# NilanEkanayake/TiTok-Video

Measured on AMD Instinct MI355X. Metric: video clips/sec encode+decode (whole node), higher is better.
Workload: dtype bf16

## Files before the change

### include/titok_hip.h

```cpp
#ifndef TITOK_HIP_H
#define TITOK_HIP_H

#include <stdint.h>

#ifdef __cplusplus
extern "C" {
#endif

#define TTV_OK 0
#define TTV_ERR_INVALID 1
#define TTV_ERR_LAUNCH 2
#define TTV_ERR_UNSUPPORTED 3

#define TTV_BF16 0
#define TTV_F32 1

#define TTV_ENCODER 0
#define TTV_DECODER 1

#define TTV_MAX_FSQ 8
#define TTV_MAX_TOKEN 64
#define TTV_MAX_CLIPS_PER_LAUNCH 64

const char* ttv_error_string(void);
// ... 68 lines not shown

int64_t ttv_mlp_pack_bytes(int inner, int next_qkv_rows);
int ttv_mlp_pack(const void* w12_folded, const void* w3, const void* out_proj, const void* next_qkv_folded, int next_qkv_rows, int inner,
                 int width, int dtype, void* mlp_packed, void* stream);
int ttv_mlp_fused(const void* x, int ldx, const void* mlp_packed, int inner, void* y, int ldy, const float* post_gain, float alpha,
                  float eps, int M, int width, int dtype, void* stream);
typedef struct ttv_next_qkv {
  void* qkv; int32_t ld;
  const float* rope_cs;
  int32_t rows;
  int32_t rope_q_end, rope_k_begin, rope_k_end;
} ttv_next_qkv;
int ttv_layer_tail_fused(const void* ao, int ldao, const float* attn_post_gain, float attn_alpha, const void* x, int ldx,
                         const void* mlp_packed, int inner, void* y, int ldy, const float* ffd_post_gain, float ffd_alpha, float eps,
                         int M, int width, int dtype, const ttv_next_qkv* next, void* stream);

int ttv_fill_const_rows(void* x, int dtype, int ld, const int32_t* rows_map, int rows, int width, const float* mask_token,
                        const float* gain, float eps, void* stream);
int ttv_decoder_embed(const void* codes, int token_size, const void* w, const void* bias, const float* mask_token, const float* gain,
                      void* x, int dtype, int ld, const int32_t* rows_map, int rows, int width, float eps, void* stream);

#define TTV_ATTN_GATE 1
#define TTV_ATTN_PAIRED 2
#define TTV_ATTN_QSCALED 4
#define TTV_ATTN_ALLFULL 8
#define TTV_ATTN_PIPE 16
#define TTV_ATTN_SPLIT3 32
#define TTV_ATTN_SPLIT_OUT 64
#define TTV_ATTN_SPLIT_IN 128
int ttv_attention(const void* qkvg, int ld, void* out, int ldo, const int32_t* cu_seqlens, const int32_t* qblocks,
// ... 434 lines not shown
  TTV_DBG_GEMM_TILE128 = 256,
  TTV_DBG_GEMM_T256 = 512,
  TTV_DBG_MLP_TILES9 = 512,
  TTV_DBG_GEMM_NO_T256 = 1024,
  TTV_DBG_MX_UNFUSED_QUANT = 2048,
  TTV_DBG_SPLIT3_NO_IMAGES = 4096,
  TTV_DBG_SPLIT3_NO_DMA = 8192,
  TTV_DBG_K256_GENERAL = 16384,
  TTV_DBG_QKV256_OFF = 32768,
  TTV_DBG_QKV256_WS = 131072,
  TTV_DBG_ENC_ALL_ROWS = 524288,
  TTV_DBG_ATTN_NO_SWP = 1048576,
  TTV_DBG_DEC_ALL_BLOCKS = 2097152,
  TTV_DBG_DEC_L0_NO_CONST = 4194304,
  TTV_DBG_ENC_LAST_QKV_ALL = 8388608,
  TTV_DBG_PATCH_EMBED_UNFUSED = 16777216
};
int ttv_debug_set(int flags);
int ttv_debug_stamps(void* device_buffer);
int ttv_prof_end(double* total_ms, int* count);

#ifdef __cplusplus
}
#endif
#endif
```

### titok_video_amd/_lib.py

```python
from __future__ import annotations

import ctypes as C
import os
import threading

import torch

from . import switches

TTV_BF16, TTV_F32 = 0, 1
TTV_ENCODER, TTV_DECODER = 0, 1
TTV_MAX_FSQ = 8
TTV_MAX_TOKEN = 64
TTV_MAX_CLIPS_PER_LAUNCH = 64
TTV_DISC_HEAD_GENERATOR, TTV_DISC_HEAD_DISCRIMINATOR = 0, 1
TTV_TAPE_STORED, TTV_TAPE_RECOMPUTE = 0, 1

DBG_NO_STORES = 1
DBG_K256_NO_PANEL_DMA = 2
DBG_MLP_NO_WEIGHT_DMA = 2
DBG_K256_NO_TILE_RELOAD = 4
DBG_MLP_NO_GEGLU = 4
DBG_K256_NO_EPILOGUE_MATH = 8
DBG_MLP_TILES8 = 8
# ... 5 lines not shown
DBG_GEMM_T256 = 512
DBG_MLP_TILES9 = 512
DBG_GEMM_NO_T256 = 1024
DBG_MX_UNFUSED_QUANT = 2048
DBG_SPLIT3_NO_IMAGES = 4096
DBG_SPLIT3_NO_DMA = 8192
DBG_K256_GENERAL = 16384
DBG_QKV256_OFF = 32768
DBG_QKV256_WS = 131072
DBG_ENC_ALL_ROWS = 524288
DBG_ATTN_NO_SWP = 1048576
DBG_DEC_ALL_BLOCKS = 2097152
DBG_DEC_L0_NO_CONST = 4194304
DBG_ENC_LAST_QKV_ALL = 8388608
DBG_PATCH_EMBED_UNFUSED = 16777216

_HERE = os.path.dirname(os.path.abspath(__file__))
LIB_PATH = switches.text("TTV_LIB_PATH") or os.path.join(_HERE, "libtitok_hip.so")

i32, i64, f32, vp = C.c_int32, C.c_int64, C.c_float, C.c_void_p


class FsqParams(C.Structure):
    _fields_ = [("n", i32), ("levels", i32 * TTV_MAX_FSQ), ("basis", i32 * TTV_MAX_FSQ),
                ("half_l", f32 * TTV_MAX_FSQ), ("offset", f32 * TTV_MAX_FSQ), ("shift", f32 * TTV_MAX_FSQ),
                ("half_width", f32 * TTV_MAX_FSQ)]


class TowerDims(C.Structure):
    _fields_ = [("kind", i32), ("dtype", i32), ("width", i32), ("layers", i32), ("q_heads", i32), ("kv_heads", i32),
# ... 150 lines not shown
    "ttv_linear_fp8_mx": (C.c_int, [vp, C.c_int, vp, vp, vp, C.c_int, vp, vp, vp, C.c_int, C.c_int, C.c_int, C.c_int, C.c_int, vp, C.c_int, C.c_int,
                                    vp, C.c_int, f32, vp]),
    "ttv_rmsnorm": (C.c_int, [vp, C.c_int, C.c_int, vp, vp, C.c_int, C.c_int, vp, vp, C.c_int, C.c_int, f32, vp]),
    "ttv_rope_apply": (C.c_int, [vp, C.c_int, C.c_int, C.c_int, C.c_int, vp, vp]),
    "ttv_linear": (C.c_int, [vp, C.c_int, vp, C.c_int, vp, vp, vp, C.c_int, C.c_int, C.c_int, C.c_int, C.c_int, vp]),
    "ttv_linear_qkv_rope": (C.c_int, [vp, C.c_int, vp, C.c_int, vp, C.c_int, C.c_int, C.c_int, C.c_int, vp, C.c_int, vp]),
    "ttv_linear_geglu": (C.c_int, [vp, C.c_int, vp, C.c_int, vp, C.c_int, C.c_int, C.c_int, C.c_int, C.c_int, vp]),
    "ttv_linear_residual": (C.c_int, [vp, C.c_int, vp, C.c_int, vp, C.c_int, f32, vp, C.c_int, C.c_int, C.c_int, C.c_int,
                                      C.c_int, C.c_int, vp]),
    "ttv_linear_residual_norm": (C.c_int, [vp, C.c_int, vp, C.c_int, vp, C.c_int, f32, vp, f32, vp, C.c_int, C.c_int, C.c_int,
                                           C.c_int, C.c_int, vp]),
    "ttv_mlp_pack_bytes": (C.c_int64, [C.c_int, C.c_int]),
    "ttv_mlp_pack": (C.c_int, [vp, vp, vp, vp, C.c_int, C.c_int, C.c_int, C.c_int, vp, vp]),
    "ttv_layer_tail_fused": (C.c_int, [vp, C.c_int, vp, f32, vp, C.c_int, vp, C.c_int, vp, C.c_int, vp, f32, f32, C.c_int, C.c_int,
                                       C.c_int, vp, vp]),
    "ttv_mlp_fused": (C.c_int, [vp, C.c_int, vp, C.c_int, vp, C.c_int, vp, f32, f32, C.c_int, C.c_int, C.c_int, vp]),
    "ttv_fill_const_rows": (C.c_int, [vp, C.c_int, C.c_int, vp, C.c_int, C.c_int, vp, vp, f32, vp]),
    "ttv_decoder_embed": (C.c_int, [vp, C.c_int, vp, vp, vp, vp, vp, C.c_int, C.c_int, vp, C.c_int, C.c_int, f32, vp]),
    "ttv_attention": (C.c_int, [vp, C.c_int, vp, C.c_int, vp, vp, C.c_int, C.c_int, C.c_int, C.c_int, C.c_int, C.c_int, vp]),
    "ttv_attention64": (C.c_int, [vp, C.c_int, vp, C.c_int, vp, vp, C.c_int, C.c_int, C.c_int, C.c_int, C.c_int, C.c_int, vp]),
    "ttv_rmsnorm_mx": (C.c_int, [vp, C.c_int, C.c_int, vp, C.c_int, C.c_int, vp, C.c_int, C.c_int, f32, vp, vp, vp, vp]),
    "ttv_attention_pv8_bytes": (C.c_int64, [C.c_int, C.c_int, C.c_int]),
    "ttv_quant_v_pv8": (C.c_int, [vp, C.c_int, vp, C.c_int, C.c_int, C.c_int, C.c_int, vp, vp]),
    "ttv_attention_pv8": (C.c_int, [vp, C.c_int, vp, C.c_int, vp, vp, C.c_int, C.c_int, C.c_int, C.c_int, C.c_int, vp, vp]),
    "ttv_attention_mxout": (C.c_int, [vp, C.c_int, vp, vp, C.c_int, vp, vp, C.c_int, C.c_int, C.c_int, vp]),
    "ttv_linear_fp8_mx_geglu_q": (C.c_int, [vp, C.c_int, vp, vp, vp, C.c_int, vp, vp, vp, vp, C.c_int, C.c_int, C.c_int, vp]),
    "ttv_row_rstd": (C.c_int, [vp, C.c_int, C.c_int, vp, C.c_int, C.c_int, f32, vp]),
    "ttv_linear_rowscale": (C.c_int, [vp, C.c_int, vp, C.c_int, vp, C.c_int, vp, C.c_int, C.c_int, vp, C.c_int, C.c_int, C.c_int, C.c_int, C.c_int, vp]),
    "ttv_patch_gather": (C.c_int, [C.POINTER(vp), vp, C.c_int, C.c_int, C.c_int, C.c_int, C.c_int, C.c_int, vp, C.c_int,
                                   C.c_int, C.c_int, vp]),
# ... 156 lines not shown
```

### titok_video_amd/csrc/ttv_api.hip

```cpp
#include <stdarg.h>
#include <stdio.h>
#include <stdlib.h>
#include <string.h>

#include "ttv_common.h"
#include "ttv_kernels.h"

static thread_local char g_err[512] = "";

void ttv_set_error(const char* fmt, ...) {
  va_list ap;
  va_start(ap, fmt);
  vsnprintf(g_err, sizeof(g_err), fmt, ap);
  va_end(ap);
}

int g_ttv_prof_class = 0;
bool ttv_sw_enc_latent_last() { static const bool v = ttv_env_flag("TTV_ENC_LATENT_LAST", true); return v; }
bool ttv_enc_latent_rows_only(const ttv_tower_dims* d, const ttv_batch* b) {
  return ttv_sw_enc_latent_last() && !(g_ttv_debug & TTV_DBG_ENC_ALL_ROWS) && d->kind == TTV_ENCODER && b->latent_rows && b->sum_tokens > 0 &&
         b->sum_tokens < b->total_rows;
}
bool ttv_sw_keel_f32sum() { static const bool v = ttv_env_flag("TTV_KEEL_F32SUM", false); return v; }
bool ttv_sw_fused_patch() { static const bool v = ttv_env_flag("TTV_FUSED_PATCH", true); return v; }
bool ttv_sw_attn_pipe() { static const bool v = ttv_env_flag("TTV_ATTN_PIPE", false); return v; }
static bool sw_dec_l0_const() { static const bool v = ttv_env_flag("TTV_DEC_L0_CONST", true); return v; }
static bool sw_enc_last_qkv_skip() { static const bool v = ttv_env_flag("TTV_ENC_LAST_QKV_SKIP", true); return v; }
float ttv_sw_attn_thr() { static const float v = ttv_env_float("TTV_ATTN_THR", 8.0f); return v; }
thread_local int g_ttv_debug = 0;
long long* g_ttv_stamps = nullptr;
static hipEvent_t* g_prof_start = nullptr;
static hipEvent_t* g_prof_stop = nullptr;
static int g_prof_cap = 0, g_prof_n = 0;

TtvProfScope::TtvProfScope(int cls, hipStream_t stream) : slot(-1), s(stream) {
  if (g_ttv_prof_class != 0 && cls == g_ttv_prof_class && g_prof_n < g_prof_cap) {
    slot = g_prof_n++;
    (void)hipEventRecord(g_prof_start[slot], s);
  }
}
TtvProfScope::~TtvProfScope() {
  if (slot >= 0) (void)hipEventRecord(g_prof_stop[slot], s);
}

struct TowerWs {
  char *x, *xn, *qkv, *ao, *h, *pa, *pb;
  char *xl, *aol;
  char *f8, *f8mx;
  float* y32;
  float* rstd;
  int64_t total;
};

static TowerWs carve(const ttv_tower_dims* d, const ttv_batch* b, char* base) {
  const int64_t e = dtype_bytes(d->dtype);
  const int64_t L = b->total_rows, P = b->sum_patches;
  const int64_t g = (int64_t)d->kv_heads * d->head_dim;
  const int64_t pd = patch_dim(d);
  int64_t off = 0;
  TowerWs w;
  auto take = [&](int64_t bytes) { char* p = base ? base + off : nullptr; off += align256(bytes); return p; };
  w.x = take(L * d->width * e);
  w.xn = take(L * d->width * e);
  w.qkv = take(L * (2 * d->width + 2 * g) * e);
  w.ao = take(L * d->width * e);
  w.y32 = (float*)take(L * d->width * 4);
  w.h = take(L * d->inner * e);
  w.pa = take(P * pd * e);
  w.pb = take(P * d->width * e);
  w.rstd = (float*)take(L * 4);
  w.xl = take((int64_t)b->sum_tokens * d->width * e);
  w.aol = take((int64_t)b->sum_tokens * d->width * e);
  w.f8 = w.f8mx = nullptr;
  if (d->dtype == TTV_BF16 && d->width != 256 && d->width % 128 == 0) {
    const int64_t wide = d->width > d->inner ? d->width : d->inner;
    w.f8 = take(L * wide);
    w.f8mx = take(L * (wide / 128 + 4) * 4);
  }
  w.total = off;
  return w;
}

static int check_dims(const ttv_tower_dims* d, const ttv_batch* b) {
  TTV_CHECK_ARG(d && b, "null dims/batch");
  TTV_CHECK_ARG(d->dtype == TTV_BF16 || d->dtype == TTV_F32, "bad dtype %d", d->dtype);
  TTV_CHECK_ARG(d->head_dim == 64 && d->width == d->q_heads * 64, "width must be q_heads*64");
  TTV_CHECK_ARG(d->width % 64 == 0 && d->width <= 1024, "width %d unsupported", d->width);
// ... 126 lines not shown
    return ttvk_gemm(EPI_RESID_NORM, o, c.s);
  }
  float* const next_rstd = want_rstd ? c.ws.rstd : nullptr;
  if (dt == TTV_BF16 && !ttv_sw_keel_f32sum()) {
    TTV_TRY(ttvk_gemm(EPI_RESID_T, o, c.s));
    TTV_TRY(ttvk_rmsnorm(cx, dt, dm, nullptr, cx, dt, dm, nullptr, post_gain, o.M, dm, d->eps, c.s, next_rstd));
  } else {
    o.y = c.ws.y32;
    TTV_TRY(ttvk_gemm(EPI_RESID_F32, o, c.s));
    TTV_TRY(ttvk_rmsnorm(c.ws.y32, TTV_F32, dm, nullptr, cx, dt, dm, nullptr, post_gain, o.M, dm, d->eps, c.s, next_rstd));
  }
  rstd_valid = want_rstd;
  return TTV_OK;
}

static bool qkv_tile_list_ok(const LayerCtx& c, const ttv_layer_weights& lw, int K, int P) {
  const ttv_tower_dims* d = c.d;
  const ttv_batch* b = c.b;
  if (d->dtype != TTV_BF16 || d->width != 256 || d->head_dim != 64 || c.split3) return false;
  if (K <= 0 || P <= 0 || K % 128 || P % 128 || (int64_t)b->n_clips * K != b->sum_tokens || (int64_t)b->n_clips * P != b->sum_patches) return false;
  if (!lw.to_qkv_pn || !lw.qkv_q_prescaled) return false;
  return ttvk_gemm_qkv_tiles_supported(d->width, d->kv_heads * d->head_dim, d->width);
}

static bool dec_l0_const_ok(const LayerCtx& c, const ttv_tower_weights* w, const ttv_dec_l0_const* l0) {
  const ttv_tower_dims* d = c.d;
  const ttv_batch* b = c.b;
  if (!l0 || !l0->rows || !sw_dec_l0_const() || (g_ttv_debug & TTV_DBG_DEC_L0_NO_CONST)) return false;
  if (d->kind != TTV_DECODER || !qkv_tile_list_ok(c, w->layers[0], l0->latent_rows, l0->patch_rows)) return false;
  if (c.pair || c.pipe || c.pv8 || !c.all_full || (b->items64 && b->n_items64 > 0)) return false;
  return ttvk_attention_takes_swp(TTV_ATTN_GATE | TTV_ATTN_QSCALED | TTV_ATTN_ALLFULL);
}

static bool enc_last_qkv_skip_ok(const LayerCtx& c, const ttv_layer_weights& lw) {
  const ttv_batch* b = c.b;
// ... 1 lines not shown
  return qkv_tile_list_ok(c, lw, b->tokens_per_clip, b->max_patches_per_clip);
}

static int run_layers(const ttv_tower_dims* d, const ttv_tower_weights* w, const ttv_batch* b, const TowerWs& ws, hipStream_t s,
                      const ttv_dec_l0_const* l0 = nullptr) {
  const int L = b->total_rows, dm = d->width, g = d->kv_heads * d->head_dim, dt = d->dtype;
  const int split3 = (dt == TTV_F32 && w->f32_split3) ? 1 : 0;
  const bool gen_ok = (dt == TTV_BF16 && dm != 256) || split3;
  static const bool s3img_env = ttv_env_flag("TTV_SPLIT3_IMAGES", true);
  const int s3img = (split3 && s3img_env && !(g_ttv_debug & TTV_DBG_SPLIT3_NO_IMAGES)) ? 1 : 0;
  const int nq = 2 * dm + 2 * g;
  const int64_t row_bytes = (int64_t)dm * dtype_bytes(dt);
  bool qkv_ready = false;
  bool rstd_valid = false;
  bool xq_valid = false;
  const bool lat_last = ttv_enc_latent_rows_only(d, b) && b->qblocks_latent && b->n_qblocks_latent > 0;
  static const bool pat_env = ttv_env_flag("TTV_DEC_PATCH_LAST", true);
  const bool pat_last = pat_env && !(g_ttv_debug & TTV_DBG_DEC_ALL_BLOCKS) && d->kind == TTV_DECODER && d->layers >= 2 && b->qblocks_patch &&
                        b->n_qblocks_patch > 0 && !split3 && !b->qblocks_paired;
  bool compacted = false;
  const bool pv8 = w->attn_pv8 != 0;
  TTV_CHECK_ARG(!pv8 || (dt == TTV_BF16 && !split3), "attn_pv8 is a bf16 inference option (not for fp32 or split-bf16 towers)");
  const LayerCtx ctx = {d, b, ws, s, split3, s3img, gen_ok, b->qblocks_paired ? TTV_ATTN_PAIRED : 0, b->qblocks_all_full ? TTV_ATTN_ALLFULL : 0,
                        ttv_sw_attn_pipe() ? TTV_ATTN_PIPE : 0, pv8};
  const bool l0_const = dec_l0_const_ok(ctx, w, l0);
  for (int i = 0; i < d->layers; ++i) {
    const ttv_layer_weights& lw = w->layers[i];
    const bool last = i == d->layers - 1;
    const bool l0c = l0_const && i == 0;
    if (dt == TTV_BF16 && dm != 256 && dm % 128 == 0 && d->inner % 128 == 0 && !ttv_sw_keel_f32sum() && lw.to_qkv_f8 && lw.to_qkv_mx && lw.w12_f8 &&
        lw.w12_mx && lw.out_proj_f8 && lw.out_proj_mx && lw.w3_f8 && lw.w3_mx &&
        !(lat_last && last)) {
      TTV_TRY(run_layer_mx(ctx, lw, i, rstd_valid, xq_valid));
      qkv_ready = false;
// ... 20 lines not shown
    else if (l0c) {
      TtvProfScope prof(TTV_KC_ATTENTION, s);
      const bool own = l0->qblocks && l0->n_qblocks > 0;
      TTV_TRY(ttvk_attention_swp(ws.qkv, nq, ws.ao, dm, b->cu_seqlens, own ? l0->qblocks : b->qblocks, own ? l0->n_qblocks : b->n_qblocks, d->q_heads,
                                 d->kv_heads, 1, s, l0->rows, l0->latent_rows, l0->state));
    } else if (pat_last && last && dt == TTV_BF16 && !ctx.pipe)
      TTV_TRY(tower_attention(ctx, q_scaled, b->qblocks_patch, b->n_qblocks_patch, ctx.all_full));
    else if (q_scaled && b->items64 && b->n_items64 > 0 && d->head_dim == 64 && !pv8)
      TTV_TRY(ttvk_attention64(ws.qkv, nq, ws.ao, dm, b->cu_seqlens, b->items64, b->n_items64, d->q_heads, d->kv_heads,
                               TTV_ATTN_GATE | TTV_ATTN_QSCALED, s));
    else
      TTV_TRY(tower_attention(ctx, q_scaled, b->qblocks, b->n_qblocks, ctx.pair | ctx.all_full | ctx.pipe));
    char* cx = ws.x;
    char* cao = ws.ao;
    int Lc = L;
    if (lat_now) {
      TTV_TRY(gather_rows(ws.x, ws.xl, b->latent_rows, b->sum_tokens, row_bytes, s));
      TTV_TRY(gather_rows(ws.ao, ws.aol, b->latent_rows, b->sum_tokens, row_bytes, s));
      cx = ws.xl; cao = ws.aol; Lc = b->sum_tokens;
      compacted = true;
    }
    static const bool use_fused_mlp = ttv_env_flag("TTV_FUSED_MLP", true);
    static const bool use_fused_qkv = ttv_env_flag("TTV_FUSED_QKV", false);
    const float alpha = keel_alpha(d, i);
    if (use_fused_mlp && ttvk_mlp_fused_supported(dt, dm, d->inner) && lw.mlp_pack) {
      MlpNextQkv nx = {};
      const bool back = use_fused_qkv && !last && lw.mlp_pack_qkv_rows == nq && nq % 64 == 0 && dm % 64 == 0 && g % 64 == 0;
      if (back) { nx.qkv = ws.qkv; nx.ld = nq; nx.rope_cs = b->rope_cs; nx.rows = nq; nx.rope_q_end = dm; nx.rope_k_begin = 2 * dm; nx.rope_k_end = 2 * dm + g; }
      TTV_TRY(ttvk_mlp_fused(cao, dm, i == 0 ? nullptr : lw.attn_post_ln, alpha, cx, dm, lw.mlp_pack, d->inner, cx, dm, i == 0 ? nullptr : lw.ffd_post_ln,
                             alpha, d->eps, Lc, back ? &nx : nullptr, s));
      qkv_ready = back;
      continue;
    }
    TTV_TRY(keel_tail(ctx, gemm_args(dt, cao, dm, lw.out_proj, dm, Lc, dm, dm, cx, dm), i, lw.attn_post_ln, gen_ok && lw.w12_pn && !f8_w12, rstd_valid));
    const PreNormW fw = {lw.ffd_norm, lw.w12, lw.w12_pn, lw.w12_f8, lw.w12_f8_scale, f8_w12};
    TTV_TRY(prenorm_proj(ctx, EPI_GEGLU, cx, Lc, fw, d->inner, ws.h, s3img, rstd_valid));
    rstd_valid = false;
    const ttv_layer_weights* nl = last ? nullptr : &w->layers[i + 1];
    const bool next_rstd = gen_ok && nl && nl->to_qkv_pn && !rows_f8(dt, dm, nl->to_qkv_f8, nl->to_qkv_f8_scale, nl->to_qkv_mx, nl->to_qkv_pn);
    TTV_TRY(keel_tail(ctx, gemm_args(dt, ws.h, d->inner, lw.w3, d->inner, Lc, dm, d->inner, cx, dm), i, lw.ffd_post_ln, next_rstd, rstd_valid));
  }
  if (compacted)
    TTV_TRY(scatter_rows(ws.xl, ws.x, b->latent_rows, b->sum_tokens, row_bytes, s));
  return TTV_OK;
}
// ... 203 lines not shown
}

int ttv_layer_tail_fused(const void* ao, int ldao, const float* attn_post_gain, float attn_alpha, const void* x, int ldx,
                         const void* mlp_packed, int inner, void* y, int ldy, const float* ffd_post_gain, float ffd_alpha, float eps,
                         int M, int width, int dtype, const ttv_next_qkv* next, void* stream) {
  if (!ttvk_mlp_fused_supported(dtype, width, inner)) {
    ttv_set_error("layer_tail_fused: only bf16, width 256, inner %% 32 == 0");
    return TTV_ERR_UNSUPPORTED;
  }
  TTV_CHECK_ARG(ao, "layer_tail_fused: null attention output");
  MlpNextQkv nx = {};
  if (next) { nx.qkv = next->qkv; nx.ld = next->ld; nx.rope_cs = next->rope_cs; nx.rows = next->rows; nx.rope_q_end = next->rope_q_end;
              nx.rope_k_begin = next->rope_k_begin; nx.rope_k_end = next->rope_k_end; }
  return ttvk_mlp_fused(ao, ldao, attn_post_gain, attn_alpha, x, ldx, mlp_packed, inner, y, ldy, ffd_post_gain, ffd_alpha, eps, M,
                        next ? &nx : nullptr, (hipStream_t)stream);
}

int ttv_fill_const_rows(void* x, int dtype, int ld, const int32_t* rows_map, int rows, int width, const float* mask_token,
                        const float* gain, float eps, void* stream) {
  TTV_CHECK_ARG(rows == 0 || (x && rows_map && mask_token && gain), "fill_const_rows: null buffer");
  return ttvk_fill_const_rows(x, dtype, ld, rows_map, rows, width, mask_token, gain, eps, (hipStream_t)stream);
}

int ttv_decoder_embed(const void* codes, int token_size, const void* w, const void* bias, const float* mask_token, const float* gain,
                      void* x, int dtype, int ld, const int32_t* rows_map, int rows, int width, float eps, void* stream) {
  TTV_CHECK_ARG(rows == 0 || (codes && w && bias && mask_token && gain && x && rows_map), "decoder_embed: null buffer");
  return ttvk_dec_embed(codes, token_size, w, bias, mask_token, gain, x, dtype, ld, rows_map, rows, width, eps, (hipStream_t)stream);
}

int ttv_attention(const void* qkvg, int ld, void* out, int ldo, const int32_t* cu_seqlens, const int32_t* qblocks, int n_qblocks,
// ... 422 lines not shown
```

### titok_video_amd/csrc/ttv_kernels.h

```cpp
#pragma once
#include <hip/hip_runtime.h>
#include <stdint.h>

#include "../../include/titok_hip.h"

int ttvk_rmsnorm(const void* in, int in_dtype, int ld_in, const int* src_rows, void* out, int out_dtype, int ld_out,
                 const int* dst_rows, const float* gain, int rows, int d, float eps, hipStream_t s, float* next_rstd = nullptr,
                 void* mx_q = nullptr, void* mx_s = nullptr,
                 int split_image = 0);
int ttvk_row_rstd(const void* in, int dtype, int ld_in, float* rstd, int rows, int d, float eps, hipStream_t s);
int ttvk_copy_rows(const void* src, int64_t ld_src_bytes, const int* src_rows, void* dst, int64_t ld_dst_bytes, const int* dst_rows, int rows,
                   int row_bytes, hipStream_t s);
int ttvk_fill_const_rows(void* x, int dtype, int ld, const int* rows_map, int rows, int d, const float* mask_token,
                         const float* gain, float eps, hipStream_t s);
int ttvk_dec_embed(const void* codes, int C, const void* w, const void* bias, const float* mask_token, const float* gain,
                   void* x, int dtype, int ld, const int* rows_map, int rows, int d, float eps, hipStream_t s);
int ttvk_fsq_forward(const ttv_fsq_params* p, const void* z, int z_dtype, int rows, void* codes, int codes_dtype, int* indices,
                     float* bounded, hipStream_t s);
int ttvk_fsq_indices_to_codes(const ttv_fsq_params* p, const int* indices, int rows, void* codes, int codes_dtype, hipStream_t s);
int ttvk_enc_tail(const void* x, int dtype, int ld, const int* rows_map, int rows, int d, const float* gain, float eps,
                  const void* w, const void* bias, int C, const ttv_fsq_params* fsq, float* z_out, void* codes, int* indices,
                  float* bounded, hipStream_t s);
int ttvk_patch_copy(bool scatter, void* const* clips, const int* clip_desc, int clip0, int n_clips, int pt, int ph, int pw,
                    int C, void* patches, int ld, int dtype, int max_patches, hipStream_t s);
// ... 109 lines not shown
int ttvk_vq_ema_update(const float* stats, float* cluster_size, float* embed_avg, float* codebook, void* copy, int copy_dtype, float* cnorm,
                       int64_t* ema_step, int N, int C, float decay, float one_minus_decay, float eps, float dead_threshold, void* workspace,
                       int64_t workspace_bytes, hipStream_t s);

bool ttvk_mlp_fused_supported(int dtype, int width, int inner);
struct MlpNextQkv {
  void* qkv; int ld;
  const float* rope_cs;
  int rows;
  int rope_q_end, rope_k_begin, rope_k_end;
};
int64_t ttvk_mlp_pack_bytes(int inner, int next_qkv_rows);
int ttvk_mlp_pack(const void* w12_folded, const void* w3, const void* wo, const void* next_qkv_folded, int next_qkv_rows, int inner,
                  void* packed, hipStream_t s);
int ttvk_mlp_fused(const void* ao, int ldao, const float* front_gain, float front_alpha, const void* x, int ldx, const void* packed,
                   int inner, void* y, int ldy, const float* post_gain, float alpha, float eps, int M, const MlpNextQkv* nq, hipStream_t s);

int ttvk_l1_loss(void* const* recon, void* const* target, void* const* grad, const int* sizes, int n_clips, int total_clips, int dtype,
                 float* loss, hipStream_t s);
int ttvk_sq_err(void* const* recon, void* const* target, const int* sizes, int n_clips, int dtype, int clamp, double* acc2, hipStream_t s);
int ttvk_rmsnorm_bwd_chain(const void* x, int ldx, const void* dy, int lddy, const float* gain1, float* dgain1, float* dx, int lddx,
                           const void* y, int y_dt, int ldy, const float* gain2, float* dgain2, float out_scale, void* cast_out, int ldc, int rows,
                           int d, float eps, int dt, hipStream_t s);
int ttvk_rmsnorm_bwd(const void* x, int x_dt, int ldx, const int* xr, const void* dy, int dy_dt, int lddy, const int* dyr,
                     const float* gain, void* dx, int dx_dt, int lddx, const int* dxr, int acc, float* dgain, int rows, int d, float eps,
                     hipStream_t s);
int ttvk_colsum(const void* a, int dt, int lda, const int* rows_map, int rows, int n, float* out, hipStream_t s);
int ttvk_sumall(const void* a, int dt, int lda, const int* rows_map, int rows, int n, const float* colw, float scale, float* out, hipStream_t s);
int ttvk_gate_fwd(const void* a, int lda, const void* gate, int ldg, void* ag, int ldo, int rows, int d, int dt, hipStream_t s);
int ttvk_gate_bwd(const void* dag, int ldd, const void* a, int lda, const void* gate, int ldg, void* da, int ldda, void* dgate, int lddg,
                  int rows, int d, int dt, float* delta, hipStream_t s);
// ... 128 lines not shown
```

### titok_video_amd/csrc/ttv_mlp.hip

```cpp
#include "ttv_common.h"
#include "ttv_kernels.h"

#define MLP_W12_CHUNKS 2048
#define MLP_W3_CHUNKS 1024
#define MLP_PANEL_CHUNKS (MLP_W12_CHUNKS + MLP_W3_CHUNKS)
#define MLP_WO_CHUNKS (4 * MLP_W12_CHUNKS)

struct MlpDev {
  const bf16_t* x; int ldx;
  const uint4* pack;
  const bf16_t* ao; int ldao;
  const float* front_gain;
  float front_alpha;
  bf16_t* qkv; int ldq;
  const float* rope_cs;
  int nqp, rope_q_end, rope_k_begin, rope_k_end;
  int I;
  bf16_t* y; int ldy;
  const float* post_gain;
  float alpha, eps;
  int M, n_tiles, debug;
  long long* stamps;
};

__global__ void k_mlp_pack(const bf16_t* __restrict__ w12f, const bf16_t* __restrict__ w3, const bf16_t* __restrict__ wo,
                           const bf16_t* __restrict__ wq, int nq_rows, int I, uint4* __restrict__ out) {
  const int np = I / 32;
  const int nqp = (nq_rows + 63) / 64;
  const int o = blockIdx.x * blockDim.x + threadIdx.x;
  if (o >= np * MLP_PANEL_CHUNKS + MLP_WO_CHUNKS + nqp * MLP_W12_CHUNKS) return;
  if (o >= np * MLP_PANEL_CHUNKS + MLP_WO_CHUNKS) {
    const int c = o - np * MLP_PANEL_CHUNKS - MLP_WO_CHUNKS, qp = c / MLP_W12_CHUNKS, cc = c - qp * MLP_W12_CHUNKS;
    const int r = cc >> 5, cp = cc & 31;
    const int ch = (cp & 16) | ((cp & 15) ^ (r & 15));
    int srow = qp * 64 + r;
    srow = srow < nq_rows ? srow : nq_rows - 1;
    const bf16_t* src = wq + (size_t)srow * 256 + (ch >> 2) * 32 + (ch & 3) * 4;
// ... 52 lines not shown
                 "s_mov_b32 m0, %0"                                                                                \
                 : "=&s"(keep__)                                                                                   \
                 : "v"(lane16), "v"(lane16 + 8192u), "s"(src_), "s"(dst_)                                          \
                 : "memory", "scc");                                                                               \
  } while (0)
#ifdef MLP_STAMPS
#define MLP_STAMP()                                                                                                \
  do {                                                                                                             \
    if (p.stamps && blockIdx.x == 0 && (wave & 3) == 0 && lane == 0 && n_stamp < 64)                               \
      p.stamps[(wave >> 2) * 64 + n_stamp++] = (long long)__builtin_readcyclecounter();                            \
  } while (0)
#else
#define MLP_STAMP() do { (void)n_stamp; } while (0)
#endif

template <int TPB, int T1, int T2, bool GELU_FIRST, bool KEEL, bool FRONT, bool BACK>
__device__ __forceinline__ void mlp_wave(const MlpDev& p, uint4* l12, uint4* l3, uint4* hb, const float* gl, int tile, int wave, int lane,
                                         int P1F, int P2F, int& n_stamp) {
  constexpr int T1A = T1 > 0 ? T1 : 1, T2A = T2 > 0 ? T2 : 1;
  const int l15 = lane & 15, kq = lane >> 4;
  const int np = p.I / 32;
  const uint32_t lane16 = lane * 16;
  const uint32_t lds_l12 = (uint32_t)(uintptr_t)(__attribute__((address_space(3))) void*)l12;
  const uint32_t lds_l3 = (uint32_t)(uintptr_t)(__attribute__((address_space(3))) void*)l3;
#define GLDS_W12(pn_, buf_)                                                                                        \
  do {                                                                                                             \
    const uint4* src__ = p.pack + ((size_t)(pn_) * MLP_PANEL_CHUNKS + wave * 64);                                  \
    const uint32_t dst__ = lds_l12 + ((buf_) * MLP_W12_CHUNKS + wave * 64) * 16;                                   \
    MLP_GLDS_4(src__, dst__);                                                                                      \
  } while (0)
#define GLDS_W3(pn_, buf_)                                                                                         \
  do {                                                                                                             \
    const uint4* src__ = p.pack + ((size_t)(pn_) * MLP_PANEL_CHUNKS + MLP_W12_CHUNKS + wave * 64);                 \
    const uint32_t dst__ = lds_l3 + ((buf_) * MLP_W3_CHUNKS + wave * 64) * 16;                                     \
    MLP_GLDS_2(src__, dst__);                                                                                      \
  } while (0)

  const int tok0 = tile * (16 * TPB) + l15;
  typedef __attribute__((address_space(1))) char gchar;
  typedef __attribute__((address_space(1))) const char gcchar;
  gcchar* const gx = (gcchar*)p.x;
  gcchar* const gao = (gcchar*)p.ao;
  gchar* const gy = (gchar*)p.y;

  MLP_STAMP();
  __syncthreads();

  bf16x8 bfr[T1A][8];
  float rstd[T1A];
  if (FRONT) {
#define GLDS_WO(wp_, buf_)                                                                                         \
  do {                                                                                                             \
    const uint4* src__ = p.pack + ((size_t)np * MLP_PANEL_CHUNKS + (wp_) * MLP_W12_CHUNKS + wave * 64);            \
    const uint32_t dst__ = lds_l12 + ((buf_) * MLP_W12_CHUNKS + wave * 64) * 16;                                   \
    MLP_GLDS_4(src__, dst__);                                                                                      \
  } while (0)
    GLDS_WO(0, 0);
    bf16x8 abf[T1A][8];
// ... 374 lines not shown
            pk[u] = __builtin_bit_cast(uint2, q);
          }
          const uint4 ox = xchg16_pair(pk[0], pk[1]);
          const u32x4_t ov = {ox.x, ox.y, ox.z, ox.w};
          if (qv[j]) *(__attribute__((address_space(1))) u32x4_t*)(qrow + ip * 64) = ov;
        }
      }
    }
#undef GLDS_WQ
    MLP_STAMP();
  }
#undef GLDS_W12
#undef GLDS_W3
}

template <int TILES, bool KEEL, bool FRONT, bool BACK>
__global__ __launch_bounds__(512, 1) void k_mlp256(MlpDev p) {
  extern __shared__ __attribute__((aligned(16))) uint4 smem[];
  uint4* const l12 = smem;
  uint4* const l3 = smem + 2 * MLP_W12_CHUNKS;
  uint4* const hb = l3 + 2 * MLP_W3_CHUNKS;
  float* const gl = reinterpret_cast<float*>(hb + 2 * TILES * 64);
  if (threadIdx.x < 256) {
    gl[threadIdx.x] = p.post_gain ? p.post_gain[threadIdx.x] : 1.0f;
    gl[256 + threadIdx.x] = (FRONT && p.front_gain) ? p.front_gain[threadIdx.x] : 1.0f;
  }
  const int lane = threadIdx.x & 63;
  const int wave = __builtin_amdgcn_readfirstlane(threadIdx.x >> 6);
  int n_stamp = 0;
  const int tile = blockIdx.x;
  if constexpr (TILES == 9) {
    if (wave < 4) mlp_wave<9, 2, 0, false, KEEL, FRONT, BACK>(p, l12, l3, hb, gl, tile, wave, lane, 2 * wave, 0, n_stamp);
    else if (wave < 6) mlp_wave<9, 0, 3, false, KEEL, FRONT, BACK>(p, l12, l3, hb, gl, tile, wave, lane, 0, 3 * (wave - 4), n_stamp);
    else if (wave == 6) mlp_wave<9, 1, 1, false, KEEL, FRONT, BACK>(p, l12, l3, hb, gl, tile, wave, lane, 8, 6, n_stamp);
    else mlp_wave<9, 0, 2, false, KEEL, FRONT, BACK>(p, l12, l3, hb, gl, tile, wave, lane, 0, 7, n_stamp);
  } else {
    constexpr int NT = TILES / 4;
    constexpr int TA = NT - NT / 2;
    const int g0 = (wave & 3) * NT;
    if (wave < 4) mlp_wave<TILES, TA, NT - TA, false, KEEL, FRONT, BACK>(p, l12, l3, hb, gl, tile, wave, lane, g0, g0 + TA, n_stamp);
    else mlp_wave<TILES, NT - TA, TA, false, KEEL, FRONT, BACK>(p, l12, l3, hb, gl, tile, wave, lane, g0 + TA, g0, n_stamp);
  }
}
#undef MLP_LD12
#undef MLP_GLDS_4
#undef MLP_GLDS_2
#undef MLP_STAMP

bool ttvk_mlp_fused_supported(int dtype, int width, int inner) { return dtype == TTV_BF16 && width == 256 && inner % 32 == 0 && inner > 0; }

int64_t ttvk_mlp_pack_bytes(int inner, int next_qkv_rows) {
  if (inner <= 0 || inner % 32 != 0 || next_qkv_rows < 0) return 0;
  return ((int64_t)(inner / 32) * MLP_PANEL_CHUNKS + MLP_WO_CHUNKS + (int64_t)((next_qkv_rows + 63) / 64) * MLP_W12_CHUNKS) * 16;
}

int ttvk_mlp_pack(const void* w12_folded, const void* w3, const void* wo, const void* next_qkv_folded, int next_qkv_rows, int inner,
                  void* packed, hipStream_t s) {
  TTV_CHECK_ARG(w12_folded && w3 && packed, "mlp_pack: null buffer");
  TTV_CHECK_ARG(inner > 0 && inner % 32 == 0, "mlp_pack: inner %% 32");
  TTV_CHECK_ARG((next_qkv_folded != nullptr) == (next_qkv_rows > 0), "mlp_pack: next_qkv weight and row count must come together");
  TTV_CHECK_ARG(((uintptr_t)w12_folded % 16 == 0) && ((uintptr_t)packed % 16 == 0) && ((uintptr_t)wo % 16 == 0) &&
                    ((uintptr_t)next_qkv_folded % 16 == 0), "mlp_pack: 16-byte alignment");
  const int total = inner / 32 * MLP_PANEL_CHUNKS + MLP_WO_CHUNKS + (next_qkv_rows + 63) / 64 * MLP_W12_CHUNKS;
  hipLaunchKernelGGL(k_mlp_pack, dim3(ttv_cdiv(total, 256)), dim3(256), 0, s, (const bf16_t*)w12_folded, (const bf16_t*)w3,
                     (const bf16_t*)wo, (const bf16_t*)next_qkv_folded, next_qkv_rows, inner, (uint4*)packed);
  TTV_CHECK_LAUNCH("mlp_pack");
  return TTV_OK;
}

int ttvk_mlp_fused(const void* ao, int ldao, const float* front_gain, float front_alpha, const void* x, int ldx, const void* packed,
                   int inner, void* y, int ldy, const float* post_gain, float alpha, float eps, int M, const MlpNextQkv* nq, hipStream_t s) {
  if (M == 0) return TTV_OK;
  TTV_CHECK_ARG(x && packed && y, "mlp_fused: null buffer");
  TTV_CHECK_ARG(inner % 32 == 0 && ldx % 8 == 0 && ldy % 8 == 0 && (!ao || ldao % 8 == 0), "mlp_fused: inner %% 32, leading dims %% 8");
  TTV_CHECK_ARG(((uintptr_t)x % 16 == 0) && ((uintptr_t)packed % 16 == 0) && ((uintptr_t)y % 16 == 0) && ((uintptr_t)ao % 16 == 0),
                "mlp_fused: 16-byte alignment");
  MlpDev d;
  d.x = (const bf16_t*)x; d.ldx = ldx; d.pack = (const uint4*)packed; d.I = inner;
  d.ao = (const bf16_t*)ao; d.ldao = ldao; d.front_gain = front_gain; d.front_alpha = front_alpha;
  d.y = (bf16_t*)y; d.ldy = ldy; d.post_gain = post_gain; d.alpha = alpha; d.eps = eps; d.M = M; d.debug = g_ttv_debug; d.stamps = g_ttv_stamps;
  d.qkv = nullptr; d.ldq = 0; d.rope_cs = nullptr; d.nqp = 0; d.rope_q_end = d.rope_k_begin = d.rope_k_end = 0;
  if (nq) {
    TTV_CHECK_ARG(nq->qkv && nq->rope_cs && nq->rows > 0 && nq->rows % 64 == 0 && nq->ld >= nq->rows && nq->ld % 4 == 0 &&
                      (uintptr_t)nq->qkv % 8 == 0, "mlp_fused: bad next-qkv arguments (rows %% 64, ld %% 4, 8-byte aligned)");
    TTV_CHECK_ARG(nq->rope_q_end % 64 == 0 && nq->rope_k_begin % 64 == 0 && nq->rope_k_end % 64 == 0, "mlp_fused: rotary ranges must be whole heads");
    d.qkv = (bf16_t*)nq->qkv; d.ldq = nq->ld; d.rope_cs = nq->rope_cs; d.nqp = nq->rows / 64;
    d.rope_q_end = nq->rope_q_end; d.rope_k_begin = nq->rope_k_begin; d.rope_k_end = nq->rope_k_end;
  }
  const int cus = 256;
  int tiles = 4;
  long best = -1;
  for (int c = 1; c <= 3; ++c) {
    const long cost = (long)ttv_cdiv(ttv_cdiv(M, 64 * c), cus) * (16 + 19 * c);
    if (best < 0 || cost < best) { best = cost; tiles = 4 * c; }
  }
  if (!nq && !(g_ttv_debug & TTV_DBG_MLP_PAIRS_ONLY)) {
    const long cost9 = (long)ttv_cdiv(ttv_cdiv(M, 144), cus) * (16 + 14 * 3);
    if (cost9 < best) { best = cost9; tiles = 9; }
  }
  if ((g_ttv_debug & TTV_DBG_MLP_TILES9) && !nq) tiles = 9;
  if (g_ttv_debug & TTV_DBG_MLP_TILES8) tiles = 8;
  if (g_ttv_debug & TTV_DBG_MLP_TILES4) tiles = 4;
  d.n_tiles = ttv_cdiv(M, 16 * tiles);
  const int grid = d.n_tiles;
  const size_t smem = (size_t)(2 * MLP_W12_CHUNKS + 2 * MLP_W3_CHUNKS + 2 * tiles * 64) * sizeof(uint4) + 2048;
  TtvProfScope prof(TTV_KC_GEMM_GEGLU, s);
#define LAUNCH_MLP(TILES_, KEEL_, FRONT_, BACK_)                                                                    \
  do {                                                                                                              \
    (void)hipFuncSetAttribute((const void*)k_mlp256<TILES_, KEEL_, FRONT_, BACK_>, hipFuncAttributeMaxDynamicSharedMemorySize, (int)smem); \
    hipLaunchKernelGGL((k_mlp256<TILES_, KEEL_, FRONT_, BACK_>), dim3(grid), dim3(512), smem, s, d);                \
  } while (0)
#define LAUNCH_MLP_F(TILES_, KEEL_)                                                                                 \
  do {                                                                                                              \
    if (ao && nq) LAUNCH_MLP(TILES_, KEEL_, true, true);                                                            \
    else if (ao) LAUNCH_MLP(TILES_, KEEL_, true, false);                                                            \
    else LAUNCH_MLP(TILES_, KEEL_, false, false);                                                                   \
  } while (0)
#define LAUNCH_MLP_9(KEEL_)                                                                                         \
  do {                                                                                                              \
    if (ao) LAUNCH_MLP(9, KEEL_, true, false);                                                                      \
    else LAUNCH_MLP(9, KEEL_, false, false);                                                                        \
  } while (0)
  TTV_CHECK_ARG(!nq || ao, "mlp_fused: the next-qkv part needs the out_proj front (ttv_layer_tail_fused)");
  if (post_gain) {
    if (tiles == 9) LAUNCH_MLP_9(true); else if (tiles == 12) LAUNCH_MLP_F(12, true); else if (tiles == 8) LAUNCH_MLP_F(8, true); else LAUNCH_MLP_F(4, true);
  } else {
    if (tiles == 9) LAUNCH_MLP_9(false); else if (tiles == 12) LAUNCH_MLP_F(12, false); else if (tiles == 8) LAUNCH_MLP_F(8, false); else LAUNCH_MLP_F(4, false);
  }
#undef LAUNCH_MLP_9
#undef LAUNCH_MLP_F
#undef LAUNCH_MLP
  TTV_CHECK_LAUNCH("mlp_fused");
  return TTV_OK;
}
```

Before: 32160.

## Run last-layer fused MLP tail only on needed row runs in encoder and decoder

Adds a row-run mode to the fused MLP/layer-tail kernel. Each block offsets its base pointers by a per-run shift, so the kernel processes only periodic row runs in place. The encoder's last layer uses this to work on latent token rows without gathering them into compact buffers, and drops the xl/aol workspaces. The decoder's last layer uses it to run the tail only on patch rows rather than all rows. This removes two gather copies and skips unneeded MLP work. In exchange it adds a new template variant, restricts tile choices to 4 or 8, and requires uniform, aligned row geometry.

```diff
diff --git a/include/titok_hip.h b/include/titok_hip.h
--- a/include/titok_hip.h
+++ b/include/titok_hip.h
@@ -106,6 +106,9 @@
 int ttv_layer_tail_fused(const void* ao, int ldao, const float* attn_post_gain, float attn_alpha, const void* x, int ldx,
                          const void* mlp_packed, int inner, void* y, int ldy, const float* ffd_post_gain, float ffd_alpha, float eps,
                          int M, int width, int dtype, const ttv_next_qkv* next, void* stream);
+int ttv_layer_tail_fused_runs(const void* ao, int ldao, const float* attn_post_gain, float attn_alpha, const void* x, int ldx,
+                              const void* mlp_packed, int inner, void* y, int ldy, const float* ffd_post_gain, float ffd_alpha, float eps,
+                              int M, int width, int dtype, int run_rows, int run_period, int run_first, int tiles, void* stream);
 
 int ttv_fill_const_rows(void* x, int dtype, int ld, const int32_t* rows_map, int rows, int width, const float* mask_token,
                         const float* gain, float eps, void* stream);
@@ -570,7 +573,9 @@
   TTV_DBG_DEC_ALL_BLOCKS = 2097152,
   TTV_DBG_DEC_L0_NO_CONST = 4194304,
   TTV_DBG_ENC_LAST_QKV_ALL = 8388608,
-  TTV_DBG_PATCH_EMBED_UNFUSED = 16777216
+  TTV_DBG_PATCH_EMBED_UNFUSED = 16777216,
+  TTV_DBG_DEC_LAST_TAIL_ALL = 33554432,
+  TTV_DBG_ENC_LAST_TAIL_COMPACT = 67108864
 };
 int ttv_debug_set(int flags);
 int ttv_debug_stamps(void* device_buffer);
diff --git a/titok_video_amd/_lib.py b/titok_video_amd/_lib.py
--- a/titok_video_amd/_lib.py
+++ b/titok_video_amd/_lib.py
@@ -43,6 +43,8 @@
 DBG_DEC_L0_NO_CONST = 4194304
 DBG_ENC_LAST_QKV_ALL = 8388608
 DBG_PATCH_EMBED_UNFUSED = 16777216
+DBG_DEC_LAST_TAIL_ALL = 33554432
+DBG_ENC_LAST_TAIL_COMPACT = 67108864
 
 _HERE = os.path.dirname(os.path.abspath(__file__))
 LIB_PATH = switches.text("TTV_LIB_PATH") or os.path.join(_HERE, "libtitok_hip.so")
@@ -223,6 +225,8 @@
     "ttv_mlp_pack": (C.c_int, [vp, vp, vp, vp, C.c_int, C.c_int, C.c_int, C.c_int, vp, vp]),
     "ttv_layer_tail_fused": (C.c_int, [vp, C.c_int, vp, f32, vp, C.c_int, vp, C.c_int, vp, C.c_int, vp, f32, f32, C.c_int, C.c_int,
                                        C.c_int, vp, vp]),
+    "ttv_layer_tail_fused_runs": (C.c_int, [vp, C.c_int, vp, f32, vp, C.c_int, vp, C.c_int, vp, C.c_int, vp, f32, f32, C.c_int, C.c_int,
+                                            C.c_int, C.c_int, C.c_int, C.c_int, C.c_int, vp]),
     "ttv_mlp_fused": (C.c_int, [vp, C.c_int, vp, C.c_int, vp, C.c_int, vp, f32, f32, C.c_int, C.c_int, C.c_int, vp]),
     "ttv_fill_const_rows": (C.c_int, [vp, C.c_int, C.c_int, vp, C.c_int, C.c_int, vp, vp, f32, vp]),
     "ttv_decoder_embed": (C.c_int, [vp, C.c_int, vp, vp, vp, vp, vp, C.c_int, C.c_int, vp, C.c_int, C.c_int, f32, vp]),
diff --git a/titok_video_amd/csrc/ttv_api.hip b/titok_video_amd/csrc/ttv_api.hip
--- a/titok_video_amd/csrc/ttv_api.hip
+++ b/titok_video_amd/csrc/ttv_api.hip
@@ -26,6 +26,8 @@
 bool ttv_sw_attn_pipe() { static const bool v = ttv_env_flag("TTV_ATTN_PIPE", false); return v; }
 static bool sw_dec_l0_const() { static const bool v = ttv_env_flag("TTV_DEC_L0_CONST", true); return v; }
 static bool sw_enc_last_qkv_skip() { static const bool v = ttv_env_flag("TTV_ENC_LAST_QKV_SKIP", true); return v; }
+static bool sw_dec_last_tail_runs() { static const bool v = ttv_env_flag("TTV_DEC_LAST_TAIL_RUNS", true); return v; }
+static bool sw_enc_last_tail_runs() { static const bool v = ttv_env_flag("TTV_ENC_LAST_TAIL_RUNS", true); return v; }
 float ttv_sw_attn_thr() { static const float v = ttv_env_float("TTV_ATTN_THR", 8.0f); return v; }
 thread_local int g_ttv_debug = 0;
 long long* g_ttv_stamps = nullptr;
@@ -41,6 +43,11 @@
 }
 TtvProfScope::~TtvProfScope() {
   if (slot >= 0) (void)hipEventRecord(g_prof_stop[slot], s);
+}
+
+static bool uniform_rows_ok(const ttv_tower_dims* d, const ttv_batch* b, int K, int P);
+static bool enc_tail_runs_geometry(const ttv_tower_dims* d, const ttv_batch* b) {
+  return sw_enc_last_tail_runs() && d->kind == TTV_ENCODER && uniform_rows_ok(d, b, b->tokens_per_clip, b->max_patches_per_clip);
 }
 
 struct TowerWs {
@@ -69,8 +76,11 @@
   w.pa = take(P * pd * e);
   w.pb = take(P * d->width * e);
   w.rstd = (float*)take(L * 4);
-  w.xl = take((int64_t)b->sum_tokens * d->width * e);
-  w.aol = take((int64_t)b->sum_tokens * d->width * e);
+  w.xl = w.aol = nullptr;
+  if (!enc_tail_runs_geometry(d, b)) {
+    w.xl = take((int64_t)b->sum_tokens * d->width * e);
+    w.aol = take((int64_t)b->sum_tokens * d->width * e);
+  }
   w.f8 = w.f8mx = nullptr;
   if (d->dtype == TTV_BF16 && d->width != 256 && d->width % 128 == 0) {
     const int64_t wide = d->width > d->inner ? d->width : d->inner;
@@ -227,11 +237,14 @@
   return TTV_OK;
 }
 
+static bool uniform_rows_ok(const ttv_tower_dims* d, const ttv_batch* b, int K, int P) {
+  if (d->dtype != TTV_BF16 || d->width != 256 || d->head_dim != 64) return false;
+  return K > 0 && P > 0 && K % 128 == 0 && P % 128 == 0 && (int64_t)b->n_clips * K == b->sum_tokens && (int64_t)b->n_clips * P == b->sum_patches;
+}
+
 static bool qkv_tile_list_ok(const LayerCtx& c, const ttv_layer_weights& lw, int K, int P) {
   const ttv_tower_dims* d = c.d;
-  const ttv_batch* b = c.b;
-  if (d->dtype != TTV_BF16 || d->width != 256 || d->head_dim != 64 || c.split3) return false;
-  if (K <= 0 || P <= 0 || K % 128 || P % 128 || (int64_t)b->n_clips * K != b->sum_tokens || (int64_t)b->n_clips * P != b->sum_patches) return false;
+  if (c.split3 || !uniform_rows_ok(d, c.b, K, P)) return false;
   if (!lw.to_qkv_pn || !lw.qkv_q_prescaled) return false;
   return ttvk_gemm_qkv_tiles_supported(d->width, d->kv_heads * d->head_dim, d->width);
 }
@@ -263,10 +276,17 @@
   bool qkv_ready = false;
   bool rstd_valid = false;
   bool xq_valid = false;
-  const bool lat_last = ttv_enc_latent_rows_only(d, b) && b->qblocks_latent && b->n_qblocks_latent > 0;
+  bool lat_last = ttv_enc_latent_rows_only(d, b) && b->qblocks_latent && b->n_qblocks_latent > 0;
+  static const bool use_fused_mlp = ttv_env_flag("TTV_FUSED_MLP", true);
+  const ttv_layer_weights& lwl = w->layers[d->layers - 1];
+  const bool tail_fused_last = use_fused_mlp && ttvk_mlp_fused_supported(dt, dm, d->inner) && lwl.mlp_pack && !split3;
+  const bool enc_runs = lat_last && tail_fused_last && enc_tail_runs_geometry(d, b) && !(g_ttv_debug & TTV_DBG_ENC_LAST_TAIL_COMPACT);
+  if (lat_last && !enc_runs && !ws.xl) lat_last = false;
   static const bool pat_env = ttv_env_flag("TTV_DEC_PATCH_LAST", true);
   const bool pat_last = pat_env && !(g_ttv_debug & TTV_DBG_DEC_ALL_BLOCKS) && d->kind == TTV_DECODER && d->layers >= 2 && b->qblocks_patch &&
                         b->n_qblocks_patch > 0 && !split3 && !b->qblocks_paired;
+  const bool dec_runs = pat_last && dt == TTV_BF16 && !ttv_sw_attn_pipe() && tail_fused_last && sw_dec_last_tail_runs() &&
+                        !(g_ttv_debug & TTV_DBG_DEC_LAST_TAIL_ALL) && uniform_rows_ok(d, b, b->tokens_per_clip, b->max_patches_per_clip);
   bool compacted = false;
   const bool pv8 = w->attn_pv8 != 0;
   TTV_CHECK_ARG(!pv8 || (dt == TTV_BF16 && !split3), "attn_pv8 is a bf16 inference option (not for fp32 or split-bf16 towers)");
@@ -317,13 +337,18 @@
     char* cx = ws.x;
     char* cao = ws.ao;
     int Lc = L;
-    if (lat_now) {
+    int run_rows = 0, run_period = 0, run_first = 0, run_tiles = 0;
+    if (lat_now && enc_runs) {
+      run_rows = b->tokens_per_clip; run_period = b->tokens_per_clip + b->max_patches_per_clip; Lc = b->sum_tokens;
+    } else if (dec_runs && last) {
+      run_rows = b->max_patches_per_clip; run_period = b->tokens_per_clip + b->max_patches_per_clip; run_first = b->tokens_per_clip;
+      run_tiles = 8; Lc = b->sum_patches;
+    } else if (lat_now) {
       TTV_TRY(gather_rows(ws.x, ws.xl, b->latent_rows, b->sum_tokens, row_bytes, s));
       TTV_TRY(gather_rows(ws.ao, ws.aol, b->latent_rows, b->sum_tokens, row_bytes, s));
       cx = ws.xl; cao = ws.aol; Lc = b->sum_tokens;
       compacted = true;
     }
-    static const bool use_fused_mlp = ttv_env_flag("TTV_FUSED_MLP", true);
     static const bool use_fused_qkv = ttv_env_flag("TTV_FUSED_QKV", false);
     const float alpha = keel_alpha(d, i);
     if (use_fused_mlp && ttvk_mlp_fused_supported(dt, dm, d->inner) && lw.mlp_pack) {
@@ -331,7 +356,7 @@
       const bool back = use_fused_qkv && !last && lw.mlp_pack_qkv_rows == nq && nq % 64 == 0 && dm % 64 == 0 && g % 64 == 0;
       if (back) { nx.qkv = ws.qkv; nx.ld = nq; nx.rope_cs = b->rope_cs; nx.rows = nq; nx.rope_q_end = dm; nx.rope_k_begin = 2 * dm; nx.rope_k_end = 2 * dm + g; }
       TTV_TRY(ttvk_mlp_fused(cao, dm, i == 0 ? nullptr : lw.attn_post_ln, alpha, cx, dm, lw.mlp_pack, d->inner, cx, dm, i == 0 ? nullptr : lw.ffd_post_ln,
-                             alpha, d->eps, Lc, back ? &nx : nullptr, s));
+                             alpha, d->eps, Lc, back ? &nx : nullptr, s, run_rows, run_period, run_first, run_tiles));
       qkv_ready = back;
       continue;
     }
@@ -565,6 +590,18 @@
               nx.rope_k_begin = next->rope_k_begin; nx.rope_k_end = next->rope_k_end; }
   return ttvk_mlp_fused(ao, ldao, attn_post_gain, attn_alpha, x, ldx, mlp_packed, inner, y, ldy, ffd_post_gain, ffd_alpha, eps, M,
                         next ? &nx : nullptr, (hipStream_t)stream);
+}
+
+int ttv_layer_tail_fused_runs(const void* ao, int ldao, const float* attn_post_gain, float attn_alpha, const void* x, int ldx,
+                              const void* mlp_packed, int inner, void* y, int ldy, const float* ffd_post_gain, float ffd_alpha, float eps,
+                              int M, int width, int dtype, int run_rows, int run_period, int run_first, int tiles, void* stream) {
+  if (!ttvk_mlp_fused_supported(dtype, width, inner)) {
+    ttv_set_error("layer_tail_fused_runs: only bf16, width 256, inner %% 32 == 0");
+    return TTV_ERR_UNSUPPORTED;
+  }
+  TTV_CHECK_ARG(ao, "layer_tail_fused_runs: null attention output");
+  return ttvk_mlp_fused(ao, ldao, attn_post_gain, attn_alpha, x, ldx, mlp_packed, inner, y, ldy, ffd_post_gain, ffd_alpha, eps, M, nullptr,
+                        (hipStream_t)stream, run_rows, run_period, run_first, tiles);
 }
 
 int ttv_fill_const_rows(void* x, int dtype, int ld, const int32_t* rows_map, int rows, int width, const float* mask_token,
diff --git a/titok_video_amd/csrc/ttv_kernels.h b/titok_video_amd/csrc/ttv_kernels.h
--- a/titok_video_amd/csrc/ttv_kernels.h
+++ b/titok_video_amd/csrc/ttv_kernels.h
@@ -147,7 +147,8 @@
 int ttvk_mlp_pack(const void* w12_folded, const void* w3, const void* wo, const void* next_qkv_folded, int next_qkv_rows, int inner,
                   void* packed, hipStream_t s);
 int ttvk_mlp_fused(const void* ao, int ldao, const float* front_gain, float front_alpha, const void* x, int ldx, const void* packed,
-                   int inner, void* y, int ldy, const float* post_gain, float alpha, float eps, int M, const MlpNextQkv* nq, hipStream_t s);
+                   int inner, void* y, int ldy, const float* post_gain, float alpha, float eps, int M, const MlpNextQkv* nq, hipStream_t s,
+                   int run_rows = 0, int run_period = 0, int run_first = 0, int want_tiles = 0);
 
 int ttvk_l1_loss(void* const* recon, void* const* target, void* const* grad, const int* sizes, int n_clips, int total_clips, int dtype,
                  float* loss, hipStream_t s);
diff --git a/titok_video_amd/csrc/ttv_mlp.hip b/titok_video_amd/csrc/ttv_mlp.hip
--- a/titok_video_amd/csrc/ttv_mlp.hip
+++ b/titok_video_amd/csrc/ttv_mlp.hip
@@ -21,6 +21,7 @@
   float alpha, eps;
   int M, n_tiles, debug;
   long long* stamps;
+  int run_rows, run_period, run_first;
 };
 
 __global__ void k_mlp_pack(const bf16_t* __restrict__ w12f, const bf16_t* __restrict__ w3, const bf16_t* __restrict__ wo,
@@ -103,7 +104,7 @@
 #define MLP_STAMP() do { (void)n_stamp; } while (0)
 #endif
 
-template <int TPB, int T1, int T2, bool GELU_FIRST, bool KEEL, bool FRONT, bool BACK>
+template <int TPB, int T1, int T2, bool GELU_FIRST, bool KEEL, bool FRONT, bool BACK, bool RUNS>
 __device__ __forceinline__ void mlp_wave(const MlpDev& p, uint4* l12, uint4* l3, uint4* hb, const float* gl, int tile, int wave, int lane,
                                          int P1F, int P2F, int& n_stamp) {
   constexpr int T1A = T1 > 0 ? T1 : 1, T2A = T2 > 0 ? T2 : 1;
@@ -128,9 +129,11 @@
   const int tok0 = tile * (16 * TPB) + l15;
   typedef __attribute__((address_space(1))) char gchar;
   typedef __attribute__((address_space(1))) const char gcchar;
-  gcchar* const gx = (gcchar*)p.x;
-  gcchar* const gao = (gcchar*)p.ao;
-  gchar* const gy = (gchar*)p.y;
+  long long rshift = 0;
+  if constexpr (RUNS) rshift = (long long)(tile * (16 * TPB) / p.run_rows) * (p.run_period - p.run_rows) + p.run_first;
+  gcchar* const gx = (gcchar*)p.x + rshift * p.ldx * 2;
+  gcchar* const gao = (gcchar*)p.ao + rshift * p.ldao * 2;
+  gchar* const gy = (gchar*)p.y + rshift * p.ldy * 2;
 
   MLP_STAMP();
   __syncthreads();
@@ -535,7 +538,7 @@
 #undef GLDS_W3
 }
 
-template <int TILES, bool KEEL, bool FRONT, bool BACK>
+template <int TILES, bool KEEL, bool FRONT, bool BACK, bool RUNS = false>
 __global__ __launch_bounds__(512, 1) void k_mlp256(MlpDev p) {
   extern __shared__ __attribute__((aligned(16))) uint4 smem[];
   uint4* const l12 = smem;
@@ -551,16 +554,16 @@
   int n_stamp = 0;
   const int tile = blockIdx.x;
   if constexpr (TILES == 9) {
-    if (wave < 4) mlp_wave<9, 2, 0, false, KEEL, FRONT, BACK>(p, l12, l3, hb, gl, tile, wave, lane, 2 * wave, 0, n_stamp);
-    else if (wave < 6) mlp_wave<9, 0, 3, false, KEEL, FRONT, BACK>(p, l12, l3, hb, gl, tile, wave, lane, 0, 3 * (wave - 4), n_stamp);
-    else if (wave == 6) mlp_wave<9, 1, 1, false, KEEL, FRONT, BACK>(p, l12, l3, hb, gl, tile, wave, lane, 8, 6, n_stamp);
-    else mlp_wave<9, 0, 2, false, KEEL, FRONT, BACK>(p, l12, l3, hb, gl, tile, wave, lane, 0, 7, n_stamp);
+    if (wave < 4) mlp_wave<9, 2, 0, false, KEEL, FRONT, BACK, RUNS>(p, l12, l3, hb, gl, tile, wave, lane, 2 * wave, 0, n_stamp);
+    else if (wave < 6) mlp_wave<9, 0, 3, false, KEEL, FRONT, BACK, RUNS>(p, l12, l3, hb, gl, tile, wave, lane, 0, 3 * (wave - 4), n_stamp);
+    else if (wave == 6) mlp_wave<9, 1, 1, false, KEEL, FRONT, BACK, RUNS>(p, l12, l3, hb, gl, tile, wave, lane, 8, 6, n_stamp);
+    else mlp_wave<9, 0, 2, false, KEEL, FRONT, BACK, RUNS>(p, l12, l3, hb, gl, tile, wave, lane, 0, 7, n_stamp);
   } else {
     constexpr int NT = TILES / 4;
     constexpr int TA = NT - NT / 2;
     const int g0 = (wave & 3) * NT;
-    if (wave < 4) mlp_wave<TILES, TA, NT - TA, false, KEEL, FRONT, BACK>(p, l12, l3, hb, gl, tile, wave, lane, g0, g0 + TA, n_stamp);
-    else mlp_wave<TILES, NT - TA, TA, false, KEEL, FRONT, BACK>(p, l12, l3, hb, gl, tile, wave, lane, g0 + TA, g0, n_stamp);
+    if (wave < 4) mlp_wave<TILES, TA, NT - TA, false, KEEL, FRONT, BACK, RUNS>(p, l12, l3, hb, gl, tile, wave, lane, g0, g0 + TA, n_stamp);
+    else mlp_wave<TILES, NT - TA, TA, false, KEEL, FRONT, BACK, RUNS>(p, l12, l3, hb, gl, tile, wave, lane, g0 + TA, g0, n_stamp);
   }
 }
 #undef MLP_LD12
@@ -590,9 +593,14 @@
 }
 
 int ttvk_mlp_fused(const void* ao, int ldao, const float* front_gain, float front_alpha, const void* x, int ldx, const void* packed,
-                   int inner, void* y, int ldy, const float* post_gain, float alpha, float eps, int M, const MlpNextQkv* nq, hipStream_t s) {
+                   int inner, void* y, int ldy, const float* post_gain, float alpha, float eps, int M, const MlpNextQkv* nq, hipStream_t s,
+                   int run_rows, int run_period, int run_first, int want_tiles) {
   if (M == 0) return TTV_OK;
   TTV_CHECK_ARG(x && packed && y, "mlp_fused: null buffer");
+  TTV_CHECK_ARG(run_rows >= 0 && (run_rows > 0 || (run_period == 0 && run_first == 0)), "mlp_fused: bad row runs");
+  TTV_CHECK_ARG(run_rows == 0 || (run_period >= run_rows && run_first >= 0 && ao && !nq),
+                "mlp_fused: row runs need run_period >= run_rows, run_first >= 0, the out_proj front and no next-qkv part");
+  TTV_CHECK_ARG(want_tiles == 0 || want_tiles == 4 || want_tiles == 8, "mlp_fused: tile variants to ask for are 4 and 8");
   TTV_CHECK_ARG(inner % 32 == 0 && ldx % 8 == 0 && ldy % 8 == 0 && (!ao || ldao % 8 == 0), "mlp_fused: inner %% 32, leading dims %% 8");
   TTV_CHECK_ARG(((uintptr_t)x % 16 == 0) && ((uintptr_t)packed % 16 == 0) && ((uintptr_t)y % 16 == 0) && ((uintptr_t)ao % 16 == 0),
                 "mlp_fused: 16-byte alignment");
@@ -620,8 +628,15 @@
     if (cost9 < best) { best = cost9; tiles = 9; }
   }
   if ((g_ttv_debug & TTV_DBG_MLP_TILES9) && !nq) tiles = 9;
+  if (run_rows) {
+    const long c4 = (long)ttv_cdiv(ttv_cdiv(M, 64), cus) * (16 + 19), c8 = (long)ttv_cdiv(ttv_cdiv(M, 128), cus) * (16 + 38);
+    tiles = c8 < c4 ? 8 : 4;
+  }
+  if (want_tiles) tiles = want_tiles;
   if (g_ttv_debug & TTV_DBG_MLP_TILES8) tiles = 8;
   if (g_ttv_debug & TTV_DBG_MLP_TILES4) tiles = 4;
+  TTV_CHECK_ARG(run_rows % (16 * tiles) == 0, "mlp_fused: run_rows %d is not a multiple of the block's %d tokens", run_rows, 16 * tiles);
+  d.run_rows = run_rows; d.run_period = run_period; d.run_first = run_first;
   d.n_tiles = ttv_cdiv(M, 16 * tiles);
   const int grid = d.n_tiles;
   const size_t smem = (size_t)(2 * MLP_W12_CHUNKS + 2 * MLP_W3_CHUNKS + 2 * tiles * 64) * sizeof(uint4) + 2048;
@@ -642,12 +657,21 @@
     if (ao) LAUNCH_MLP(9, KEEL_, true, false);                                                                      \
     else LAUNCH_MLP(9, KEEL_, false, false);                                                                        \
   } while (0)
+#define LAUNCH_MLP_RUNS(TILES_, KEEL_)                                                                              \
+  do {                                                                                                              \
+    (void)hipFuncSetAttribute((const void*)k_mlp256<TILES_, KEEL_, true, false, true>, hipFuncAttributeMaxDynamicSharedMemorySize, (int)smem); \
+    hipLaunchKernelGGL((k_mlp256<TILES_, KEEL_, true, false, true>), dim3(grid), dim3(512), smem, s, d);            \
+  } while (0)
   TTV_CHECK_ARG(!nq || ao, "mlp_fused: the next-qkv part needs the out_proj front (ttv_layer_tail_fused)");
-  if (post_gain) {
+  if (run_rows) {
+    if (post_gain) { if (tiles == 8) LAUNCH_MLP_RUNS(8, true); else LAUNCH_MLP_RUNS(4, true); }
+    else { if (tiles == 8) LAUNCH_MLP_RUNS(8, false); else LAUNCH_MLP_RUNS(4, false); }
+  } else if (post_gain) {
     if (tiles == 9) LAUNCH_MLP_9(true); else if (tiles == 12) LAUNCH_MLP_F(12, true); else if (tiles == 8) LAUNCH_MLP_F(8, true); else LAUNCH_MLP_F(4, true);
   } else {
     if (tiles == 9) LAUNCH_MLP_9(false); else if (tiles == 12) LAUNCH_MLP_F(12, false); else if (tiles == 8) LAUNCH_MLP_F(8, false); else LAUNCH_MLP_F(4, false);
   }
+#undef LAUNCH_MLP_RUNS
 #undef LAUNCH_MLP_9
 #undef LAUNCH_MLP_F
 #undef LAUNCH_MLP
```

Result: no change. 31880 (-0.9%).
